# IC3Net/IC3Net

Measured on AMD Instinct MI355X. Metric: env-steps/sec (agents x envs x steps), rollout hot path, higher is better.
Workload: dtype f32

## Files before the change

### ic3net_amd/csrc/gates_bwd.hip

```cpp
#include <hip/hip_runtime.h>

#include "ic3_common.hpp"

namespace ic3 {

typedef float gb_f32x4 __attribute__((ext_vector_type(4)));
typedef float gb_f32x16 __attribute__((ext_vector_type(16)));
typedef unsigned int gb_u32x4 __attribute__((ext_vector_type(4)));

struct GatesBwdArgs {
    float* xh;
    const float* h_prev;
    const float* wq;
    const void* wq3;
    const float* bias;
    const float* c_prev;
    const float* dh;
    const float* dc;
    float* dgates;
    float* dc_prev;
    float* dbias;
    int ldx, R, accumulate;
    const void* wb3;
    float* dxh;
    const float* gates;
    const float* row_live;
    const float* row_keep;
    const float* dhead;
    const float* w_heads;
    int OT;
};

__device__ __forceinline__ __amdgpu_buffer_rsrc_t gb_rsrc(const void* base, long long bytes)
{
    const uint32_t n = bytes <= 0 ? 0u : (bytes > 0xffffffffll ? 0xffffffffu : (uint32_t)bytes);
    return __builtin_amdgcn_make_buffer_rsrc(const_cast<void*>(base), 0, n, 0x00020000);
}
__device__ __forceinline__ gb_f32x4 gb_load4(__amdgpu_buffer_rsrc_t r, int voff, int soff)
{
    return __builtin_bit_cast(gb_f32x4, __builtin_amdgcn_raw_buffer_load_b128(r, voff, soff, 0));
}
__device__ __forceinline__ float gb_load1(__amdgpu_buffer_rsrc_t r, int voff, int soff)
{
    return __builtin_bit_cast(float, __builtin_amdgcn_raw_buffer_load_b32(r, voff, soff, 0));
}
__device__ __forceinline__ void gb_store1(float v, __amdgpu_buffer_rsrc_t r, int voff, int soff)
{
    __builtin_amdgcn_raw_buffer_store_b32(__builtin_bit_cast(int, v), r, voff, soff, 0);
}

__device__ __forceinline__ void gb_mfma(gb_f32x16& acc, float x, float y)
{
    acc = __builtin_amdgcn_mfma_f32_32x32x2f32(x, y, acc, 0, 0, 0);
}

typedef __bf16 gb_bf16x2 __attribute__((ext_vector_type(2)));
typedef float gb_f32x2 __attribute__((ext_vector_type(2)));
__device__ __forceinline__ void gb_split_pair(gb_f32x2 x, unsigned& p1, unsigned& p2, unsigned& p3)
{
    const gb_bf16x2 h1 = __builtin_convertvector(x, gb_bf16x2);
    const gb_f32x2 r1 = x - __builtin_convertvector(h1, gb_f32x2);
    const gb_bf16x2 h2 = __builtin_convertvector(r1, gb_bf16x2);
    const gb_f32x2 r2 = r1 - __builtin_convertvector(h2, gb_f32x2);
    const gb_bf16x2 h3 = __builtin_convertvector(r2, gb_bf16x2);
    p1 = __builtin_bit_cast(unsigned, h1);
    p2 = __builtin_bit_cast(unsigned, h2);
    p3 = __builtin_bit_cast(unsigned, h3);
}
__device__ __forceinline__ void gb_split_frag(gb_f32x4 x0, gb_f32x4 x1, gb_u32x4 (&out)[3])
{
    unsigned p[3][4];
    gb_split_pair(gb_f32x2{ x0[0], x0[1] }, p[0][0], p[1][0], p[2][0]);
    gb_split_pair(gb_f32x2{ x0[2], x0[3] }, p[0][1], p[1][1], p[2][1]);
    gb_split_pair(gb_f32x2{ x1[0], x1[1] }, p[0][2], p[1][2], p[2][2]);
    gb_split_pair(gb_f32x2{ x1[2], x1[3] }, p[0][3], p[1][3], p[2][3]);
#pragma unroll
    for (int pl = 0; pl < 3; ++pl) out[pl] = gb_u32x4{ p[pl][0], p[pl][1], p[pl][2], p[pl][3] };
}
__device__ __forceinline__ void gb_mfma_bf16(gb_f32x16& acc, gb_u32x4 x, gb_u32x4 y)
{
    typedef __bf16 gb_bf16x8 __attribute__((ext_vector_type(8)));
    acc = __builtin_amdgcn_mfma_f32_32x32x16_bf16(__builtin_bit_cast(gb_bf16x8, x), __builtin_bit_cast(gb_bf16x8, y), acc, 0, 0, 0);
}

template <int H, int SPLIT = 0, int GIVEN = 0>
__global__ __launch_bounds__(2 * H, (H <= 128) ? 2 : 1) void lstm_gates_bwd_kernel(const GatesBwdArgs a)
{
    static_assert(!GIVEN || SPLIT == 1, "recorded gates: the split instantiation (its dx product)");
    constexpr int K = 2 * H, LDA = K + 4, LDA4 = LDA / 4, NT = 2 * H, KB = K / 8, K4 = K / 4, RING = 8;
    static_assert(KB % 2 == 0 && KB >= 4, "K / 8 must be even");
    IC3_DYNAMIC_LDS(float, smem);
    float* const As = smem;
    gb_f32x4* const As4 = reinterpret_cast<gb_f32x4*>(smem);
    float* const slb = As + 64 * LDA;
    float* const sdh = slb + 4 * H;
    const int tid = threadIdx.x, lane = tid & 63, w = tid >> 6, li = lane & 31, lh = lane >> 5;
    const int col = 32 * w + li;
    const long long r0 = (long long)blockIdx.x * 64;
    const int rows = (int)((a.R - r0) < 64 ? (a.R - r0) : 64);

    if constexpr (GIVEN != 0) {
        if (a.dhead) {
            const __amdgpu_buffer_rsrc_t rdd = gb_rsrc(a.dhead + r0 * a.OT, (long long)rows * a.OT * 4);
            for (int idx = tid; idx < 64 * 16; idx += NT) {
                const int row = idx >> 4, o = idx & 15;
                sdh[idx] = o < a.OT ? gb_load1(rdd, (row * a.OT + o) * 4, 0) : 0.0f;
            }
        }
        if (a.xh && a.h_prev) {
            const __amdgpu_buffer_rsrc_t rx = gb_rsrc(a.xh + r0 * a.ldx, ((long long)(rows - 1) * a.ldx + K) * 4);
            const __amdgpu_buffer_rsrc_t rhp = gb_rsrc(a.h_prev + r0 * H, (long long)rows * H * 4);
            constexpr int H4 = H / 4, PERH = 64 * H4 / NT;
#pragma unroll
            for (int i = 0; i < PERH; ++i) {
                const int idx = tid + i * NT, row = idx / H4, c4 = idx - row * H4;
                gb_f32x4 v = gb_load4(rhp, (row * H + 4 * c4) * 4, 0);
                if (a.row_live) v *= (row < rows ? a.row_live[r0 + row] : 0.0f);
                __builtin_amdgcn_raw_buffer_store_b128(__builtin_bit_cast(gb_u32x4, v), rx, (row * a.ldx + H + 4 * c4) * 4, 0, 0);
            }
        }
    } else {
        const __amdgpu_buffer_rsrc_t rx = gb_rsrc(a.xh + r0 * a.ldx, ((long long)(rows - 1) * a.ldx + K) * 4);
        constexpr int PER = 64 * K4 / NT;
        const __amdgpu_buffer_rsrc_t rhp = gb_rsrc(a.h_prev ? a.h_prev + r0 * H : a.xh, a.h_prev ? (long long)rows * H * 4 : 0);
        const bool from_h = a.h_prev != nullptr;
        gb_f32x4 v[PER];
#pragma unroll
        for (int i = 0; i < PER; ++i) {
            const int idx = tid + i * NT, row = idx / K4, c4 = idx - row * K4;
            if (from_h && c4 >= H / 4) {
                v[i] = gb_load4(rhp, (row * H + 4 * c4 - H) * 4, 0);
                __builtin_amdgcn_raw_buffer_store_b128(__builtin_bit_cast(gb_u32x4, v[i]), rx, (row * a.ldx + 4 * c4) * 4, 0, 0);
            } else {
                v[i] = gb_load4(rx, (row * a.ldx + 4 * c4) * 4, 0);
            }
        }
        if (tid < H) reinterpret_cast<gb_f32x4*>(slb)[tid] = reinterpret_cast<const gb_f32x4*>(a.bias)[tid];
#pragma unroll
        for (int i = 0; i < PER; ++i) {
            const int idx = tid + i * NT, row = idx / K4, c4 = idx - row * K4;
            As4[row * LDA4 + c4] = v[i];
        }
    }
    const int voff = (4 * lh * H + col) * 4;
    float cold[2][16];
    const __amdgpu_buffer_rsrc_t rc = gb_rsrc(a.c_prev + r0 * H, (long long)rows * H * 4);
    if constexpr (SPLIT == 0) {
#pragma unroll
        for (int rt = 0; rt < 2; ++rt)
#pragma unroll
            for (int reg = 0; reg < 16; ++reg)
                cold[rt][reg] = gb_load1(rc, voff, (32 * rt + (reg & 3) + 8 * (reg >> 2)) * H * 4);
    }
    gb_f32x16 acc[2][4];
#pragma unroll
    for (int rt = 0; rt < 2; ++rt)
#pragma unroll
        for (int gt = 0; gt < 4; ++gt)
#pragma unroll
            for (int i = 0; i < 16; ++i) acc[rt][gt][i] = 0.0f;
    if constexpr (GIVEN != 0) {
    } else if constexpr (SPLIT != 0) {
        constexpr int KB16 = K / 16, NWv = H / 32;
        const __amdgpu_buffer_rsrc_t rg3 = gb_rsrc(a.wq3, (long long)3 * K * 4 * H * 2);
        const int g3lane = (w * 64 + lane) * 16;
        constexpr int GSTRIDE = NWv * 64 * 16;
        auto wq3 = [&](int pl, int kb, int gt) {
            return __builtin_amdgcn_raw_buffer_load_b128(rg3, g3lane, ((pl * KB16 + kb) * 4 + gt) * GSTRIDE, 0);
        };
        gb_u32x4 bq[3][4];
#pragma unroll
        for (int pl = 0; pl < 3; ++pl)
#pragma unroll
            for (int gt = 0; gt < 4; ++gt) bq[pl][gt] = wq3(pl, 0, gt);
        __syncthreads();
        auto block3 = [&](auto refill_c, int kb) {
            constexpr bool REFILL = decltype(refill_c)::value;
            gb_u32x4 ap[2][3];
            {
                const gb_f32x4* s0 = As4 + li * LDA4 + 4 * kb + 2 * lh;
                const gb_f32x4* s1 = As4 + (32 + li) * LDA4 + 4 * kb + 2 * lh;
                gb_split_frag(s0[0], s0[1], ap[0]);
                gb_split_frag(s1[0], s1[1], ap[1]);
            }
#pragma unroll
            for (int pb = 0; pb < 3; ++pb)
#pragma unroll
                for (int gt = 0; gt < 4; ++gt) {
#pragma unroll
                    for (int pa = 2; pa >= 0; --pa) {
                        gb_mfma_bf16(acc[0][gt], ap[0][pa], bq[pb][gt]);
                        gb_mfma_bf16(acc[1][gt], ap[1][pa], bq[pb][gt]);
                    }
                    if constexpr (REFILL) bq[pb][gt] = wq3(pb, kb + 1, gt);
                    __builtin_amdgcn_sched_barrier(0);
                }
        };
#pragma unroll 1
        for (int kb = 0; kb < KB16 - 1; ++kb) block3(std::true_type{}, kb);
        block3(std::false_type{}, KB16 - 1);
        __builtin_amdgcn_sched_barrier(0);
    } else {
        const __amdgpu_buffer_rsrc_t rgw = gb_rsrc(a.wq, (long long)K * 4 * H * 4);
        const int glane = (4 * lh * H + col) * 16;
        auto wq = [&](int kb, int j) { return gb_load4(rgw, glane, (8 * kb + j) * (H * 16)); };
        gb_f32x4 wk[RING];
    #pragma unroll
        for (int i = 0; i < RING; ++i) wk[i] = wq(i >> 2, i & 3);
        __syncthreads();
        auto block = [&](auto sb_c, auto refill_c, int kb) {
            constexpr int SB = decltype(sb_c)::value;
            constexpr bool REFILL = decltype(refill_c)::value;
            const gb_f32x4 a0 = As4[li * LDA4 + 2 * kb + lh];
            const gb_f32x4 a1 = As4[(32 + li) * LDA4 + 2 * kb + lh];
    #pragma unroll
            for (int j = 0; j < 4; ++j) {
    #pragma unroll
                for (int gt = 0; gt < 4; ++gt) {
                    gb_mfma(acc[0][gt], a0[j], wk[SB + j][gt]);
                    gb_mfma(acc[1][gt], a1[j], wk[SB + j][gt]);
                }
                if constexpr (REFILL) wk[SB + j] = wq(kb + RING / 4, j);
                __builtin_amdgcn_sched_barrier(0);
            }
        };
        constexpr std::integral_constant<int, 0> s0{};
        constexpr std::integral_constant<int, 4> s1{};
    #pragma unroll 1
        for (int kb = 0; kb < KB - 2; kb += 2) {
            block(s0, std::true_type{}, kb);
            block(s1, std::true_type{}, kb + 1);
        }
        block(s0, std::false_type{}, KB - 2);
        block(s1, std::false_type{}, KB - 1);
        __builtin_amdgcn_sched_barrier(0);
    }

    const float bi = GIVEN ? 0.f : slb[col], bf = GIVEN ? 0.f : slb[H + col], bg = GIVEN ? 0.f : slb[2 * H + col], bo = GIVEN ? 0.f : slb[3 * H + col];
    const bool dx = SPLIT != 0 && a.dxh != nullptr;
    float keep_g[2][16], keep_o[2][16];
    const bool heads_in = GIVEN != 0 && a.dhead != nullptr;
    if (dx || heads_in) __syncthreads();
    float wh[16] = {};
    if constexpr (GIVEN != 0) {
        if (heads_in) {
            const __amdgpu_buffer_rsrc_t rwh = gb_rsrc(a.w_heads, (long long)a.OT * H * 4);
#pragma unroll
            for (int o = 0; o < 16; ++o) wh[o] = gb_load1(rwh, (o * H + col) * 4, 0);
        }
    }
    const long long nrec = (long long)rows * H * 4;
    const __amdgpu_buffer_rsrc_t rdh = gb_rsrc(a.dh ? a.dh + r0 * H : a.c_prev, a.dh ? nrec : 0);
    const __amdgpu_buffer_rsrc_t rdc = gb_rsrc(a.dc ? a.dc + r0 * H : a.c_prev, a.dc ? nrec : 0);
    const __amdgpu_buffer_rsrc_t rdp = gb_rsrc(a.dc_prev + r0 * H, nrec);
    const __amdgpu_buffer_rsrc_t rdg = gb_rsrc(a.dgates + r0 * 4 * H, 4 * nrec);
    const int goff = (4 * lh * 4 * H + col) * 4;
    const __amdgpu_buffer_rsrc_t rgin = gb_rsrc(GIVEN ? a.gates + r0 * 4 * H : a.c_prev, GIVEN ? 4 * nrec : 0);
    const bool cuts = GIVEN != 0 && (a.row_live != nullptr || a.row_keep != nullptr);
    const __amdgpu_buffer_rsrc_t rlive = gb_rsrc(a.row_live ? a.row_live + r0 : a.c_prev, a.row_live ? (long long)rows * 4 : 0);
    const __amdgpu_buffer_rsrc_t rkeep = gb_rsrc(a.row_keep ? a.row_keep + r0 : a.c_prev, a.row_keep ? (long long)rows * 4 : 0);
    float si = 0.f, sf = 0.f, sg = 0.f, so = 0.f;
#pragma unroll
    for (int rt = 0; rt < 2; ++rt) {
        float dhv[16], dcv[16], gin[GIVEN ? 4 : 1][16];
#pragma unroll
        for (int reg = 0; reg < 16; ++reg) {
            const int lc = 32 * rt + (reg & 3) + 8 * (reg >> 2);
            dhv[reg] = gb_load1(rdh, voff, lc * H * 4);
            dcv[reg] = gb_load1(rdc, voff, lc * H * 4);
            if constexpr (SPLIT != 0) cold[rt][reg] = gb_load1(rc, voff, lc * H * 4);
            if constexpr (GIVEN != 0) {
#pragma unroll
                for (int k = 0; k < 4; ++k) gin[k][reg] = gb_load1(rgin, goff, lc * 4 * H * 4 + k * H * 4);
            }
        }
#pragma unroll
        for (int reg = 0; reg < 16; ++reg) {
            const int lc = 32 * rt + (reg & 3) + 8 * (reg >> 2);
            float i, f, gt, o;
            if constexpr (GIVEN != 0) {
                i = gin[0][reg], f = gin[1][reg], gt = gin[2][reg], o = gin[3][reg];
                if (heads_in) {
                    const gb_f32x4* dr = reinterpret_cast<const gb_f32x4*>(sdh + (lc + 4 * lh) * 16);
                    float s = dhv[reg];
#pragma unroll
                    for (int q = 0; q < 4; ++q) {
                        if (4 * q >= a.OT) break;
                        const gb_f32x4 dv = dr[q];
                        s = __builtin_fmaf(dv[0], wh[4 * q], s);
                        s = __builtin_fmaf(dv[1], wh[4 * q + 1], s);
                        s = __builtin_fmaf(dv[2], wh[4 * q + 2], s);
                        s = __builtin_fmaf(dv[3], wh[4 * q + 3], s);
                    }
                    dhv[reg] = s;
                }
                if (cuts) {
                    const int lrow = lc + 4 * lh;
                    if (a.row_live) cold[rt][reg] *= gb_load1(rlive, lrow * 4, 0);
                    if (a.row_keep) dcv[reg] *= gb_load1(rkeep, lrow * 4, 0);
                }
            } else {
                i = fast_sigmoid(acc[rt][0][reg] + bi), f = fast_sigmoid(acc[rt][1][reg] + bf);
                gt = fast_tanh(acc[rt][2][reg] + bg), o = fast_sigmoid(acc[rt][3][reg] + bo);
            }
            const float c0 = cold[rt][reg];
            const float tc = fast_tanh(__builtin_fmaf(f, c0, i * gt));
            const float dct = dcv[reg] + dhv[reg] * o * (1.0f - tc * tc);
            const float di = dct * gt * i * (1.0f - i), df = dct * c0 * f * (1.0f - f);
            const float dg = dct * i * (1.0f - gt * gt), dO = dhv[reg] * tc * o * (1.0f - o);
            gb_store1(di, rdg, goff, lc * 4 * H * 4);
            gb_store1(df, rdg, goff, lc * 4 * H * 4 + H * 4);
            gb_store1(dg, rdg, goff, lc * 4 * H * 4 + 2 * H * 4);
            gb_store1(dO, rdg, goff, lc * 4 * H * 4 + 3 * H * 4);
            gb_store1(dct * f, rdp, voff, lc * H * 4);
            if constexpr (SPLIT != 0) {
                if (dx) {
                    const int lr = lc + 4 * lh;
                    As[lr * LDA + col] = di;
                    As[lr * LDA + H + col] = df;
                    keep_g[rt][reg] = dg;
                    keep_o[rt][reg] = dO;
                }
            }
            si += di;
            sf += df;
            sg += dg;
            so += dO;
        }
    }
    if constexpr (SPLIT != 0) {
        if (dx) {
            constexpr int KB16B = 4 * H / 16, NCT = 2 * H / 32, KBH = K / 16;
            const __amdgpu_buffer_rsrc_t rwb = gb_rsrc(a.wb3, (long long)3 * 4 * H * 2 * H * 2);
            const int wu = __builtin_amdgcn_readfirstlane(w);
            auto wb = [&](int pl, int kg, int ct) __attribute__((always_inline)) {
                return __builtin_amdgcn_raw_buffer_load_b128(rwb, lane * 16, ((pl * KB16B + kg) * NCT + 2 * wu + ct) * 1024, 0);
            };
            gb_u32x4 bq2[3][2];
#pragma unroll
            for (int pl = 0; pl < 3; ++pl)
#pragma unroll
                for (int ct = 0; ct < 2; ++ct) bq2[pl][ct] = wb(pl, 0, ct);
#pragma unroll
            for (int rt = 0; rt < 2; ++rt)
#pragma unroll
                for (int ct = 0; ct < 2; ++ct)
#pragma unroll
                    for (int i = 0; i < 16; ++i) acc[rt][ct][i] = 0.0f;
            auto blockdx = [&](int kb, int kg) __attribute__((always_inline)) {
                gb_u32x4 ap[2][3];
                const gb_f32x4* s0 = As4 + li * LDA4 + 4 * kb + 2 * lh;
                const gb_f32x4* s1 = As4 + (32 + li) * LDA4 + 4 * kb + 2 * lh;
                gb_split_frag(s0[0], s0[1], ap[0]);
                gb_split_frag(s1[0], s1[1], ap[1]);
#pragma unroll
                for (int pb = 0; pb < 3; ++pb)
#pragma unroll
                    for (int ct = 0; ct < 2; ++ct) {
#pragma unroll
                        for (int pa = 2; pa >= 0; --pa) {
                            gb_mfma_bf16(acc[0][ct], ap[0][pa], bq2[pb][ct]);
                            gb_mfma_bf16(acc[1][ct], ap[1][pa], bq2[pb][ct]);
                        }
                        if (kg + 1 < KB16B) bq2[pb][ct] = wb(pb, kg + 1, ct);
                        __builtin_amdgcn_sched_barrier(0);
                    }
            };
            __syncthreads();
#pragma unroll 1
            for (int kb = 0; kb < KBH; ++kb) blockdx(kb, kb);
            __syncthreads();
#pragma unroll
            for (int rt = 0; rt < 2; ++rt)
#pragma unroll
                for (int reg = 0; reg < 16; ++reg) {
                    const int lr = 32 * rt + (reg & 3) + 8 * (reg >> 2) + 4 * lh;
                    As[lr * LDA + col] = keep_g[rt][reg];
                    As[lr * LDA + H + col] = keep_o[rt][reg];
                }
            __syncthreads();
#pragma unroll 1
            for (int kb = 0; kb < KBH; ++kb) blockdx(kb, KBH + kb);
            const __amdgpu_buffer_rsrc_t rdx = gb_rsrc(a.dxh + r0 * K, (long long)rows * K * 4);
#pragma unroll
            for (int rt = 0; rt < 2; ++rt)
#pragma unroll
                for (int ct = 0; ct < 2; ++ct)
#pragma unroll
                    for (int reg = 0; reg < 16; ++reg) {
                        const int lr = 32 * rt + (reg & 3) + 8 * (reg >> 2) + 4 * lh;
                        gb_store1(acc[rt][ct][reg], rdx, (lr * K + 64 * w + 32 * ct + li) * 4, 0);
                    }
        }
    }
    if (a.dbias) {
        si += __shfl_xor(si, 32);
        sf += __shfl_xor(sf, 32);
        sg += __shfl_xor(sg, 32);
        so += __shfl_xor(so, 32);
        if (lh == 0) {
            float* d = a.dbias + (size_t)blockIdx.x * 4 * H + col;
            if (a.accumulate) {
                d[0] += si;
                d[H] += sf;
                d[2 * H] += sg;
                d[3 * H] += so;
            } else {
                d[0] = si;
                d[H] = sf;
                d[2 * H] = sg;
                d[3 * H] = so;
            }
        }
    }
}

}

extern "C" int ic3_lstm_gates_backward_supported(int H) { return H == 64 || H == 128 || H == 256; }

static int gates_backward_impl(float* xh, int ldx, const float* h_prev, const float* lstm_wp, const void* lstm_wp3, const float* bias,
                               const float* c_prev, const float* dh, const float* dc, float* dgates, float* dc_prev,
                               float* dbias_partials, int accumulate, const void* wb3, float* dxh, int R, int H, ic3_stream stream,
                               const float* gates = nullptr, const float* row_live = nullptr, const float* row_keep = nullptr,
                               const float* dhead = nullptr, const float* w_heads = nullptr, int OT = 0);

extern "C" int ic3_lstm_gates_backward(float* xh, int ldx, const float* h_prev, const float* lstm_wp, const void* lstm_wp3, const float* bias, const float* c_prev,
                                       const float* dh, const float* dc, float* dgates, float* dc_prev, float* dbias_partials,
                                       int accumulate, int R, int H, ic3_stream stream)
{
    return gates_backward_impl(xh, ldx, h_prev, lstm_wp, lstm_wp3, bias, c_prev, dh, dc, dgates, dc_prev, dbias_partials, accumulate,
                               nullptr, nullptr, R, H, stream);
}

extern "C" int ic3_lstm_gates_backward_dx(float* xh, int ldx, const float* h_prev, const float* lstm_wp, const void* lstm_wp3,
                                          const void* lstm_wp3_bwd, const float* bias, const float* c_prev, const float* dh,
                                          const float* dc, float* dgates, float* dc_prev, float* dbias_partials, int accumulate,
                                          float* dxh, int R, int H, ic3_stream stream)
{
    if (!lstm_wp3 || !lstm_wp3_bwd || !dxh)
        return ic3::fail(-22, "ic3_lstm_gates_backward_dx: needs the split planes of both products (lstm_wp3, lstm_wp3_bwd) and dxh");
    if (H != 64 && H != 128) return ic3::fail(-38, "ic3_lstm_gates_backward_dx: hid_size 64 / 128");
    return gates_backward_impl(xh, ldx, h_prev, lstm_wp, lstm_wp3, bias, c_prev, dh, dc, dgates, dc_prev, dbias_partials, accumulate,
                               lstm_wp3_bwd, dxh, R, H, stream);
}

extern "C" int ic3_lstm_gates_backward_given(const float* gates, float* xh, int ldx, const float* h_prev, const void* lstm_wp3_bwd,
                                             const float* c_prev, const float* dh, const float* dc, float* dgates, float* dc_prev,
                                             float* dbias_partials, int accumulate, float* dxh, const float* row_live,
                                             const float* row_keep, const float* dhead, const float* w_heads, int OT, int R, int H,
                                             ic3_stream stream)
{
    if (!gates) return ic3::fail(-22, "ic3_lstm_gates_backward_given: null gates");
    if ((dhead == nullptr) != (w_heads == nullptr) || (dhead && (OT < 1 || OT > 16)))
        return ic3::fail(-22, "ic3_lstm_gates_backward_given: dhead [R][OT] and w_heads [OT][H] come together, 1 <= OT <= 16");
    if (row_keep && !dc) return ic3::fail(-22, "ic3_lstm_gates_backward_given: row_keep scales dc");
    if ((lstm_wp3_bwd == nullptr) != (dxh == nullptr))
        return ic3::fail(-22, "ic3_lstm_gates_backward_given: lstm_wp3_bwd and dxh come together");
    if (H != 64 && H != 128 && H != 256) return ic3::fail(-38, "ic3_lstm_gates_backward_given: hid_size 64 / 128 / 256");
    if ((xh == nullptr) != (h_prev == nullptr))
        return ic3::fail(-22, "ic3_lstm_gates_backward_given: xh and h_prev come together (the copy into xh's h half) or not at all");
    return gates_backward_impl(xh, xh ? ldx : 2 * H, h_prev, nullptr, nullptr, nullptr, c_prev, dh, dc, dgates, dc_prev, dbias_partials,
                               accumulate, lstm_wp3_bwd, dxh, R, H, stream, gates, row_live, row_keep, dhead, w_heads, OT);
}

template <int H>
static auto gates_bwd_kernel_of(bool given, bool split)
{
    return given ? ic3::lstm_gates_bwd_kernel<H, 1, 1> : split ? ic3::lstm_gates_bwd_kernel<H, 1> : ic3::lstm_gates_bwd_kernel<H, 0>;
}

static int gates_backward_impl(float* xh, int ldx, const float* h_prev, const float* lstm_wp, const void* lstm_wp3, const float* bias,
                               const float* c_prev, const float* dh, const float* dc, float* dgates, float* dc_prev,
                               float* dbias_partials, int accumulate, const void* wb3, float* dxh, int R, int H, ic3_stream stream,
                               const float* gates, const float* row_live, const float* row_keep, const float* dhead,
                               const float* w_heads, int OT)
{
    using namespace ic3;
    if ((!gates && (!xh || !lstm_wp || !bias)) || !c_prev || (!dh && !gates) || !dgates || !dc_prev || R <= 0)
        return fail(-22, "ic3_lstm_gates_backward: null argument");
    if (!ic3_lstm_gates_backward_supported(H)) return fail(-38, "ic3_lstm_gates_backward: needs hid_size 64 / 128 / 256");
    if (ldx < 2 * H || (ldx & 3)) return fail(-22, "ic3_lstm_gates_backward: ldx must be a multiple of 4, >= 2 * hid_size");
    if ((long long)R * (ldx > 4 * H ? ldx : 4 * H) * 4 >= (1ll << 32))
        return fail(-22, "ic3_lstm_gates_backward: R * 4H floats must stay below 4 GB (32-bit buffer offsets)");
    const GatesBwdArgs a{ xh, h_prev, lstm_wp, lstm_wp3, bias, c_prev, dh, dc, dgates, dc_prev, dbias_partials, ldx, R, accumulate, wb3, dxh, gates, row_live, row_keep, dhead, w_heads, OT };
    const int tiles = (R + 63) / 64;
    const size_t lds = ((size_t)64 * (2 * H + 4) + 4 * H + (gates ? 64 * 16 : 0)) * sizeof(float);
    hipStream_t s = (hipStream_t)stream;
    const bool given = gates != nullptr, split = lstm_wp3 != nullptr;
    const auto kernel = H == 256 ? gates_bwd_kernel_of<256>(given, split)
                                 : H == 128 ? gates_bwd_kernel_of<128>(given, split) : gates_bwd_kernel_of<64>(given, split);
    if (const int rc = launch_kernel(kernel, dim3(tiles), dim3(2 * H), lds, s, a); rc < 0) return rc;
    return tiles;
}
```

Before: 283.7 million.

## Stage dgates as pre-split bf16 MFMA planes in LDS per gate

Instead of writing fp32 gate gradients into the shared A tile and splitting them into bf16 fragments inside every MFMA block, each thread now pairs values across lanes, splits them once into three bf16 planes, and writes them in MFMA fragment order. The dx GEMM then runs over four gate passes, each reading ready fragments with one vector LDS load per plane. The aim is to drop the repeated split work and strided LDS reads from the inner loop. The cost is more barriers (one per gate instead of two halves), extra cross-lane shuffles, and more registers held to keep three gates' gradients live.

```diff
diff --git a/ic3net_amd/csrc/gates_bwd.hip b/ic3net_amd/csrc/gates_bwd.hip
--- a/ic3net_amd/csrc/gates_bwd.hip
+++ b/ic3net_amd/csrc/gates_bwd.hip
@@ -238,9 +238,26 @@
 
     const float bi = GIVEN ? 0.f : slb[col], bf = GIVEN ? 0.f : slb[H + col], bg = GIVEN ? 0.f : slb[2 * H + col], bo = GIVEN ? 0.f : slb[3 * H + col];
     const bool dx = SPLIT != 0 && a.dxh != nullptr;
-    float keep_g[2][16], keep_o[2][16];
+    float keep[3][2][16];
     const bool heads_in = GIVEN != 0 && a.dhead != nullptr;
     if (dx || heads_in) __syncthreads();
+    unsigned* const planes = reinterpret_cast<unsigned*>(smem);
+    const int odd = li & 1, pc0 = col & ~1;
+    const int pbase = (pc0 >> 4) * 1536 + (odd + 4 * lh + 32 * ((pc0 >> 3) & 1)) * 4 + ((pc0 & 7) >> 1);
+    auto plane_pair = [&](int rt, int pr, float d0, float d1) __attribute__((always_inline)) {
+        const float got = __shfl_xor(odd ? d0 : d1, 1);
+        const gb_f32x2 x = odd ? gb_f32x2{ got, d1 } : gb_f32x2{ d0, got };
+        unsigned p1, p2, p3;
+        gb_split_pair(x, p1, p2, p3);
+        unsigned* const dst = planes + pbase + rt * 768 + (((2 * pr) & 3) + 8 * (pr >> 1)) * 4;
+        dst[0] = p1;
+        dst[256] = p2;
+        dst[512] = p3;
+    };
+    auto plane_write = [&](int rt, const float (&d)[16]) __attribute__((always_inline)) {
+#pragma unroll
+        for (int pr = 0; pr < 8; ++pr) plane_pair(rt, pr, d[2 * pr], d[2 * pr + 1]);
+    };
     float wh[16] = {};
     if constexpr (GIVEN != 0) {
         if (heads_in) {
@@ -262,7 +279,7 @@
     float si = 0.f, sf = 0.f, sg = 0.f, so = 0.f;
 #pragma unroll
     for (int rt = 0; rt < 2; ++rt) {
-        float dhv[16], dcv[16], gin[GIVEN ? 4 : 1][16];
+        float dhv[16], dcv[16], gin[GIVEN ? 4 : 1][16], di_even = 0.f;
 #pragma unroll
         for (int reg = 0; reg < 16; ++reg) {
             const int lc = 32 * rt + (reg & 3) + 8 * (reg >> 2);
@@ -315,11 +332,18 @@
             gb_store1(dct * f, rdp, voff, lc * H * 4);
             if constexpr (SPLIT != 0) {
                 if (dx) {
-                    const int lr = lc + 4 * lh;
-                    As[lr * LDA + col] = di;
-                    As[lr * LDA + H + col] = df;
-                    keep_g[rt][reg] = dg;
-                    keep_o[rt][reg] = dO;
+                    float ki = di, kf = df, kg = dg, ko = dO;
+                    if constexpr (GIVEN == 0) {
+                        IC3_OPAQUE_VGPR(ki);
+                        IC3_OPAQUE_VGPR(kf);
+                        IC3_OPAQUE_VGPR(kg);
+                        IC3_OPAQUE_VGPR(ko);
+                    }
+                    if (reg & 1) plane_pair(rt, reg >> 1, di_even, ki);
+                    else di_even = ki;
+                    keep[0][rt][reg] = kf;
+                    keep[1][rt][reg] = kg;
+                    keep[2][rt][reg] = ko;
                 }
             }
             si += di;
@@ -330,7 +354,8 @@
     }
     if constexpr (SPLIT != 0) {
         if (dx) {
-            constexpr int KB16B = 4 * H / 16, NCT = 2 * H / 32, KBH = K / 16;
+            constexpr int KB16B = 4 * H / 16, NCT = 2 * H / 32, KBG = H / 16;
+            const gb_u32x4* const planes4 = reinterpret_cast<const gb_u32x4*>(smem);
             const __amdgpu_buffer_rsrc_t rwb = gb_rsrc(a.wb3, (long long)3 * 4 * H * 2 * H * 2);
             const int wu = __builtin_amdgcn_readfirstlane(w);
             auto wb = [&](int pl, int kg, int ct) __attribute__((always_inline)) {
@@ -349,10 +374,10 @@
                     for (int i = 0; i < 16; ++i) acc[rt][ct][i] = 0.0f;
             auto blockdx = [&](int kb, int kg) __attribute__((always_inline)) {
                 gb_u32x4 ap[2][3];
-                const gb_f32x4* s0 = As4 + li * LDA4 + 4 * kb + 2 * lh;
-                const gb_f32x4* s1 = As4 + (32 + li) * LDA4 + 4 * kb + 2 * lh;
-                gb_split_frag(s0[0], s0[1], ap[0]);
-                gb_split_frag(s1[0], s1[1], ap[1]);
+#pragma unroll
+                for (int rt = 0; rt < 2; ++rt)
+#pragma unroll
+                    for (int pl = 0; pl < 3; ++pl) ap[rt][pl] = planes4[((2 * kb + rt) * 3 + pl) * 64 + lane];
 #pragma unroll
                 for (int pb = 0; pb < 3; ++pb)
 #pragma unroll
@@ -366,21 +391,17 @@
                         __builtin_amdgcn_sched_barrier(0);
                     }
             };
-            __syncthreads();
+#pragma unroll
+            for (int gate = 0; gate < 4; ++gate) {
+                if (gate > 0) {
+                    __syncthreads();
+                    plane_write(0, keep[gate - 1][0]);
+                    plane_write(1, keep[gate - 1][1]);
+                }
+                __syncthreads();
 #pragma unroll 1
-            for (int kb = 0; kb < KBH; ++kb) blockdx(kb, kb);
-            __syncthreads();
-#pragma unroll
-            for (int rt = 0; rt < 2; ++rt)
-#pragma unroll
-                for (int reg = 0; reg < 16; ++reg) {
-                    const int lr = 32 * rt + (reg & 3) + 8 * (reg >> 2) + 4 * lh;
-                    As[lr * LDA + col] = keep_g[rt][reg];
-                    As[lr * LDA + H + col] = keep_o[rt][reg];
-                }
-            __syncthreads();
-#pragma unroll 1
-            for (int kb = 0; kb < KBH; ++kb) blockdx(kb, KBH + kb);
+                for (int kb = 0; kb < KBG; ++kb) blockdx(kb, gate * KBG + kb);
+            }
             const __amdgpu_buffer_rsrc_t rdx = gb_rsrc(a.dxh + r0 * K, (long long)rows * K * 4);
 #pragma unroll
             for (int rt = 0; rt < 2; ++rt)
```

Result: no change. 282.5 million (-0.4%).
